# aayush9400/3D-Condtional-Stable-Diffusion

Measured on AMD Instinct MI355X. Metric: latent volumes/sec at 32^3x8ch T=1000 DDPM, higher is better.
Workload: dtype f32 (f16 hi+lo x3 MFMA, f32 accumulate)

## Files before the change

### 3d-condtional-stable-diffusion_amd/_lib.py

```python
from __future__ import annotations

import ctypes as C
import os

_HERE = os.path.dirname(os.path.abspath(__file__))
LIB_PATH = os.environ.get("DM3D_LIB") or os.path.join(_HERE, "csrc", "libdm3d_hip.so")

ACT_NONE, ACT_RELU, ACT_SILU = 0, 1, 2
ABI_VERSION = 111
PREC_F32, PREC_H3 = 0, 1
WL_TAP, WL_PAIR = 0, 1
FMT_F32, FMT_H2 = 0, 1
COUT_PAD, CIN_PAD = 64, 16

_f32p = C.c_void_p
_i32p = C.c_void_p


class ConvDesc(C.Structure):
    _fields_ = [
        ("x1", _f32p), ("x2", _f32p), ("c1", C.c_int32), ("c2", C.c_int32), ("batch", C.c_int32),
        ("in_d", C.c_int32), ("in_h", C.c_int32), ("in_w", C.c_int32), ("upsample", C.c_int32),
        ("ksize", C.c_int32), ("stride", C.c_int32), ("wpk", _f32p), ("bias", _f32p),
        ("pro_scale", _f32p), ("pro_shift", _f32p), ("vec", _f32p), ("vec_idx", _i32p), ("vec_ld", C.c_int32),
# ... 216 lines not shown
GRADNORM_PARTIAL_BLOCKS = 1024
PAIR_PARTIAL_BLOCKS = 64
SSIM_TILE = 32
EDT_MAX_EXTENT = 512
EDT_SURFACE, EDT_FOREGROUND = 0, 1
CCL_MAX_EXTENT = 512
CCL_BLOCK_VOXELS = 1024
CCL_LARGEST, CCL_MIN_SIZE, CCL_FILL_HOLES = 0, 1, 2
SPLINE_MAX_EXTENT = 512
RESAMPLE_F32, RESAMPLE_F64 = 0, 1
NORM_PARTIAL_BLOCKS = 256
AUG_PARTIAL_BLOCKS = 256
STREAM_AUGMENT = 0xA063
MSSSIM_TILE = (32, 16, 32)

SIGNATURES = {
    "dm3d_version": (C.c_int, []),
    "dm3d_last_error": (C.c_char_p, []),
    "dm3d_device_ok": (C.c_int, []),
    "dm3d_packed_weight_elems": (C.c_int64, [C.c_int32, C.c_int32, C.c_int32]),
    "dm3d_pack_weights": (C.c_int, [_f32p, C.c_int32, C.c_int32, C.c_int32, _f32p, _f32p, C.c_void_p]),
    "dm3d_packed_weight_h3_bytes": (C.c_int64, [C.c_int32, C.c_int32, C.c_int32]),
    "dm3d_pack_weights_h3": (C.c_int, [_f32p, C.c_int32, C.c_int32, C.c_int32, C.c_int32, _f32p, C.c_void_p, C.c_void_p]),
    "dm3d_packed_weight_h3p_bytes": (C.c_int64, [C.c_int32, C.c_int32, C.c_int32]),
    "dm3d_pack_weights_h3p": (C.c_int, [_f32p, C.c_int32, C.c_int32, C.c_int32, C.c_int32, _f32p, C.c_void_p, C.c_int32, C.c_void_p]),
    "dm3d_packed_weight_h3w_bytes": (C.c_int64, [C.c_int32, C.c_int32]),
    "dm3d_pack_weights_h3w": (C.c_int, [_f32p, C.c_int32, C.c_int32, C.c_int32, _f32p, C.c_void_p, C.c_void_p]),
    "dm3d_packed_weight_skip_h3p_bytes": (C.c_int64, [C.c_int32, C.c_int32]),
    "dm3d_pack_weights_skip_h3p": (C.c_int, [_f32p, C.c_int32, C.c_int32, C.c_int32, C.c_void_p, C.c_void_p]),
    "dm3d_pack_weights_skip_h3f": (C.c_int, [_f32p, C.c_int32, C.c_int32, C.c_int32, C.c_void_p, C.c_void_p]),
    "dm3d_conv_scratch_bytes": (C.c_int64, [C.POINTER(ConvDesc)]),
    "dm3d_conv_split_counter_words": (C.c_int32, [C.POINTER(ConvDesc)]),
    "dm3d_conv_tile_form": (C.c_int32, [C.POINTER(ConvDesc)]),
    "dm3d_conv_weight_layout": (C.c_int32, [C.c_int32, C.c_int32, C.c_int32, C.c_int32, C.c_int32]),
    "dm3d_attention_workspace_bytes": (C.c_int64, [C.c_int32, C.c_int32, C.c_int32]),
    "dm3d_attention": (C.c_int, [C.POINTER(AttentionDesc), C.c_void_p, C.c_void_p]),
    "dm3d_attention_group": (C.c_int, [C.POINTER(AttentionDesc), C.c_int32, C.c_void_p, C.c_void_p]),
    "dm3d_packed_weight_up_elems": (C.c_int64, [C.c_int32, C.c_int32]),
    "dm3d_pack_weights_up": (C.c_int, [_f32p, C.c_int32, C.c_int32, _f32p, C.c_void_p]),
    "dm3d_packed_weight_up_h3_bytes": (C.c_int64, [C.c_int32, C.c_int32]),
    "dm3d_pack_weights_up_h3": (C.c_int, [_f32p, C.c_int32, C.c_int32, C.c_int32, C.c_void_p, C.c_void_p]),
    "dm3d_pack_weights_convt": (C.c_int, [_f32p, C.c_int32, C.c_int32, _f32p, C.c_void_p]),
    "dm3d_pack_weights_convt_h3": (C.c_int, [_f32p, C.c_int32, C.c_int32, C.c_int32, C.c_void_p, C.c_void_p]),
    "dm3d_conv3d_ndhwc": (C.c_int, [C.POINTER(ConvDesc), C.c_void_p]),
    "dm3d_gemm_tn": (C.c_int, [C.POINTER(GemmDesc), C.c_void_p]),
    "dm3d_gemm_tn_group": (C.c_int, [C.POINTER(GemmDesc), C.c_int32, C.c_void_p]),
    "dm3d_mlp_fused": (C.c_int, [C.POINTER(MlpDesc), C.c_void_p]),
    "dm3d_pack_mlp_weights": (C.c_int, [C.c_void_p, C.c_int32, C.c_int32, C.c_void_p, C.c_void_p]),
    "dm3d_attn_front": (C.c_int, [C.POINTER(AttnFrontDesc), C.c_void_p]),
    "dm3d_pack_front_weights": (C.c_int, [C.c_void_p, C.c_int32, C.c_int32, C.c_void_p, C.c_void_p]),
    "dm3d_split_h2": (C.c_int, [_f32p, C.c_int64, C.c_int32, C.c_int64, C.c_int32, C.c_void_p, C.c_int64, C.c_void_p]),
    "dm3d_layernorm3_h2": (C.c_int, [_f32p, C.c_int64, C.c_int32, C.c_float] + [_f32p] * 9 + [C.c_void_p]),
    "dm3d_softmax_rows_h2": (C.c_int, [_f32p, C.c_int64, C.c_int32, C.c_int64, C.c_void_p]),
    "dm3d_layernorm3": (C.c_int, [_f32p, C.c_int64, C.c_int32, C.c_float] + [_f32p] * 9 + [C.c_void_p]),
    "dm3d_groupnorm_stats": (C.c_int, [_f32p, C.c_int32, C.c_int64, C.c_int32, C.c_void_p, C.c_int32, C.c_int32, C.c_void_p]),
    "dm3d_groupnorm_finalize": (C.c_int, [C.c_void_p, C.c_int32, C.c_int64, C.c_int32, C.c_int32, C.c_float, _f32p, _f32p, _f32p,
                                           _f32p, C.c_void_p]),
    "dm3d_groupnorm_finalize2": (C.c_int, [C.c_void_p, C.c_int32, C.c_void_p, C.c_int32, C.c_int32, C.c_int64, C.c_int32, C.c_float, _f32p, _f32p,
                                          _f32p, _f32p, C.c_void_p]),
    "dm3d_groupnorm_partials": (C.c_int, [_f32p, C.c_int32, C.c_int64, C.c_int32, C.c_void_p, C.c_void_p]),
    "dm3d_groupnorm_partials_bytes": (C.c_int64, [C.c_int32, C.c_int64, C.c_int32]),
    "dm3d_affine_act_batched": (C.c_int, [_f32p, _f32p, C.c_int32, C.c_int64, C.c_int32, _f32p, _f32p, C.c_int32, C.c_void_p]),
    "dm3d_softmax_rows": (C.c_int, [_f32p, C.c_int64, C.c_int32, C.c_int64, C.c_void_p]),
    "dm3d_affine_act": (C.c_int, [_f32p, _f32p, C.c_int64, C.c_int32, _f32p, _f32p, C.c_int32, C.c_void_p]),
    "dm3d_ddpm_update": (C.c_int, [C.POINTER(DdpmDesc), C.c_void_p]),
    "dm3d_ddim_update": (C.c_int, [C.POINTER(DdimDesc), C.c_void_p]),
# ... 117 lines not shown
```

### 3d-condtional-stable-diffusion_amd/csrc/dm3d_conv.hip

```cpp
#include <algorithm>
#include <cstdlib>
#include "dm3d_conv_args.h"
#include <math.h>

namespace {

template <int TD, int TH, int TW, int S, int KS, int WM, int WN>
__global__ __launch_bounds__(256, 2) void conv3d_igemm_f32(const ConvArgs p) {
    constexpr int CK = 16, LDV = CK + 4, NT = 64;
    constexpr int TM = TD * TH * TW;
    constexpr int HD = (TD - 1) * S + KS, HH = (TH - 1) * S + KS, HW = (TW - 1) * S + KS;
    constexpr int HVOX = HD * HH * HW;
    constexpr int TAPS = KS * KS * KS;
    constexpr int MR = TM / WM / 32, NR = NT / WN / 32;
    constexpr int NTHR = WM * WN * 64;
    constexpr int NSLOT = (HVOX * 4 + NTHR - 1) / NTHR;
    static_assert(NTHR == 256, "kernel assumes 4 waves");
    static_assert(TM % (WM * 32) == 0 && NT % (WN * 32) == 0, "tile split");

    extern __shared__ __attribute__((aligned(16))) float smem[];
    float* lds_in = smem;
    float* lds_w = smem + HVOX * LDV;

    const int tid = threadIdx.x;
// ... 148 lines not shown
#pragma unroll
            for (int r = 0; r < 16; ++r) {
                float v = acc[mr][nr][r] + add;
                if (p.relu) v = fmaxf(v, 0.0f);
                if (p.prelu) { const float al = p.prelu[o[r] % sample_elems]; v = v > 0.0f ? v : al * v; }
                if (p.res) v += rv[r];
                if (p.relu_out) v = fmaxf(v, 0.0f);
                if (ok[r]) p.out[o[r]] = v;
            }
        }
    }
}

template <int TD, int TH, int TW, int S, int KS, int WM, int WN>
int launch_conv(ConvArgs& a, hipStream_t st) {
    constexpr int LDV = 20;
    constexpr int HVOX = ((TD - 1) * S + KS) * ((TH - 1) * S + KS) * ((TW - 1) * S + KS);
    constexpr size_t lds = (size_t)(HVOX * LDV + 2 * 64 * LDV) * sizeof(float);
    a.bd = (a.od + TD - 1) / TD;
    a.bh = (a.oh + TH - 1) / TH;
    a.bw = (a.ow + TW - 1) / TW;
    static std::atomic<bool> attr_set[64] = {};
    if (int dev = dm3d_dyn_lds(lds, attr_set, "conv", &conv3d_igemm_f32<TD, TH, TW, S, KS, WM, WN>); dev < 0) return dev;
    dim3 grid((unsigned)(a.batch * a.bd * a.bh * a.bw), (unsigned)(a.coutpad / 64), a.parity ? 8u : 1u);
    hipLaunchKernelGGL((conv3d_igemm_f32<TD, TH, TW, S, KS, WM, WN>), grid, dim3(256), lds, st, a);
    return dm3d_launch_check("conv3d_igemm_f32");
}

}


struct ConvKnobs {
    bool pair_off; int ksplit_mode; long split_wgs, split_target; int split_minchunks, split_maxparts; bool wino_split_off;
    int v3_td; long wide_wgs; bool wino_off; int wino_minchunks, wino_split_minchunks;
};
static ConvKnobs conv_knobs() {
    auto num = [](const char* name, long dflt) { const char* e = getenv(name); return e ? atol(e) : dflt; };
    auto zero = [](const char* name) { const char* e = getenv(name); return e && e[0] == '0'; };
    static const ConvKnobs once = {
        zero("DM3D_CONV_PAIR"),
        (int)num("DM3D_CONV_KSPLIT", -1),
        num("DM3D_CONV_SPLIT_WGS", 256),
        num("DM3D_CONV_SPLIT_TARGET", 512),
        (int)num("DM3D_CONV_SPLIT_MINCHUNKS", 2),
        (int)num("DM3D_CONV_SPLIT_MAXPARTS", 16),
        zero("DM3D_CONV_WINO_SPLIT"),
        0, 0, false, 0, 0};
    ConvKnobs k = once;
    k.v3_td = (int)num("DM3D_CONV_V3_TD", 0);
    k.wide_wgs = num("DM3D_CONV_WIDE_WGS", 512);
    k.wino_off = zero("DM3D_CONV_WINO");
    k.wino_minchunks = (int)num("DM3D_CONV_WINO_MINCHUNKS", 2);
    k.wino_split_minchunks = (int)num("DM3D_CONV_WINO_SPLIT_MINCHUNKS", 16);
    return k;
}

static long split_tiles(const ConvArgs& a, int td) {
    return (long)a.batch * ((a.od + td - 1) / td) * ((a.oh + 7) / 8) * ((a.ow + 7) / 8) * (a.coutpad / 64) * (a.parity ? 8 : 1);
}

static int direct_ksplit(const ConvArgs& a, const ConvKnobs& K) {
    const long wgs = split_tiles(a, 4);
    if (K.ksplit_mode == 0 || wgs > K.split_wgs || a.nchunks < 4) return 1;
    int best = 1;
    for (int d = 2; d <= K.split_maxparts; ++d) {
        if (a.nchunks % d != 0 || a.nchunks / d < K.split_minchunks) continue;
        best = d;
        if (wgs * d >= K.split_target) break;
    }
    return best;
}

static int winograd_ksplit(const ConvArgs& a, const ConvKnobs& K) {
    if (K.wino_split_off || a.nchunks % 2 != 0 || a.nchunks < K.wino_split_minchunks) return 1;
    const long wgs = (long)a.batch * (a.od / 8) * (a.oh / 8) * (a.ow / 8) * (a.coutpad / 64);
    return wgs <= 128 ? 2 : 1;
}

static bool winograd_serves(const ConvArgs& a, int which, int ksplit, const ConvKnobs& K) {
    if (!a.wpk_wino || which != DM3D_CONV_K3S1 || a.parity || a.cout <= 32) return false;
    if (a.s_npairs > 0) {
        if (!a.swpk_f) return false;
        const long long svox = (long long)a.batch * a.ind * a.inh * a.inw;
        if (svox * (a.sc1 > a.sc2 ? a.sc1 : a.sc2) * 4 >= (1ll << 32)) return false;
    }
    if (a.od % 8 != 0 || a.oh % 8 != 0 || a.ow % 8 != 0 || a.padz != 1 || a.pady != 1 || a.padx != 1) return false;
    if (K.wino_off || a.nchunks < K.wino_minchunks) return false;
// ... 39 lines not shown
    a.prelu = d->prelu_alpha; a.relu_out = d->relu_out;
    a.scratch = d->scratch; a.scratch_bytes = d->scratch_bytes;
    a.split_counters = d->split_counters; a.split_counter_words = d->split_counter_words;
    a.range_flag = d->range_flag; a.range_limit = d->range_limit > 0.0f ? d->range_limit : 65504.0f;
    a.wpk_wino = d->wpk_wino;
    a.x_h2 = d->x1_fmt == DM3D_FMT_H2; a.out_h2 = d->out_fmt == DM3D_FMT_H2;
    a.post_scale = d->post_scale; a.post_shift = d->post_shift;
    if (d->skip_wpk) {
        a.sx1 = d->skip_x1; a.sx2 = d->skip_x2; a.sc1 = d->skip_c1; a.sc2 = d->skip_c2; a.swpk = d->skip_wpk;
        a.s_npairs = (int)(dm3d_round_up(d->skip_c1 + d->skip_c2, 32) / 32);
        a.swpk_f = d->skip_wpk_frag;
    }
    a.batch = d->batch;
    a.out_scale = d->precision == DM3D_PREC_H3 ? ldexpf(1.0f, -d->w_exp) : 1.0f;
    if (par_mode) a.w_parity_stride = d->precision == DM3D_PREC_H3
        ? dm3d_packed_weight_h3_bytes(8, cin, d->cout) / 2 : dm3d_packed_weight_elems(8, cin, d->cout);
    a.gn_stats = d->gn_stats;
    r.a = a;
    r.which = par_mode ? DM3D_CONV_UP
                       : (d->ksize == 1 ? DM3D_CONV_K1 : (d->ksize == 4 ? DM3D_CONV_K4S2 : (d->stride == 2 ? DM3D_CONV_K3S2 : DM3D_CONV_K3S1)));

    if (d->precision != DM3D_PREC_H3) { r.family = DM3D_CONV_FAM_F32; return r; }
    if (dm3d_conv_weight_layout(d->ksize, d->stride, d->upsample, d->transpose, d->cout) != DM3D_WL_PAIR) { r.family = DM3D_CONV_FAM_TAP; return r; }
    const bool wino_geometry = r.which == DM3D_CONV_K3S1 && a.cout > 32 && a.od % 8 == 0 && a.oh % 8 == 0 && a.ow % 8 == 0;
    const int ks_direct = direct_ksplit(a, K), ks_wino = wino_geometry ? winograd_ksplit(a, K) : 1;
    auto bytes = [&](int td, int ks) { return split_tiles(a, td) * ks * (int64_t)(td * 8 * 8 * 64) * (int64_t)sizeof(float); };
    if (winograd_serves(a, r.which, a.split_counters ? ks_wino : 1, K)) {
        r.family = DM3D_CONV_FAM_WINO; r.td = 8; r.nct = 4;
        r.ksplit = a.split_counters ? ks_wino : 1;
    } else {
        r.family = DM3D_CONV_FAM_V3;
        r.nct = (r.which == DM3D_CONV_K3S1 && a.cout <= 32) ? (a.cout <= 16 ? 1 : 2) : 4;
        r.td = r.nct != 4 ? 4 : direct_td(a, K);
        r.ksplit = (r.td == 4 && a.split_counters) ? ks_direct : 1;
    }
    r.tiles = split_tiles(a, r.td);
    r.tile_floats = (long)r.td * 8 * 8 * 64;
    if (r.ksplit > 1) { r.need_words = r.tiles; r.need_bytes = bytes(r.td, r.ksplit); }
    if (d->batch <= 0 || d->cout <= 0 || d->in_d <= 0 || d->in_h <= 0 || d->in_w <= 0) return r;
    if (ks_direct > 1) { r.can_words = split_tiles(a, 4); r.can_bytes = bytes(4, ks_direct); }
    if (ks_wino > 1) { r.can_words = std::max(r.can_words, split_tiles(a, 8)); r.can_bytes = std::max(r.can_bytes, bytes(8, ks_wino)); }
    return r;
}

static int conv_validate(const dm3d_conv_desc* d) {
    DM3D_REQUIRE(d != nullptr, "conv: null descriptor");
    DM3D_REQUIRE(d->x1 && d->wpk && d->out, "conv: x1/wpk/out must be non-null");
    DM3D_REQUIRE(d->ksize == 1 || d->ksize == 3 || (d->ksize == 4 && d->stride == 2), "conv: ksize %d not in {1,3} (4 needs stride 2)", d->ksize);
    DM3D_REQUIRE(d->stride == 1 || d->stride == 2, "conv: stride %d not in {1,2}", d->stride);
    DM3D_REQUIRE(!d->transpose || (d->ksize == 4 && d->stride == 2 && !d->upsample), "conv: transpose needs ksize 4, stride 2, no upsample");
    DM3D_REQUIRE(!(d->upsample && d->stride != 1), "conv: upsample requires stride 1");
    DM3D_REQUIRE(!(d->ksize == 1 && (d->stride != 1 || d->upsample)), "conv: ksize 1 supports stride 1 without upsample only");
    DM3D_REQUIRE(d->batch > 0 && d->in_d > 0 && d->in_h > 0 && d->in_w > 0 && d->cout > 0, "conv: non-positive extent");
    DM3D_REQUIRE(d->c1 > 0 && d->c1 % 4 == 0 && d->c2 >= 0 && d->c2 % 4 == 0, "conv: c1=%d c2=%d must be multiples of 4", d->c1, d->c2);
    DM3D_REQUIRE((d->c2 == 0) == (d->x2 == nullptr), "conv: x2 and c2 must be given together");
    DM3D_REQUIRE(d->c2 == 0 || d->c1 % 16 == 0, "conv: with a second input c1=%d must be a multiple of 16", d->c1);
    DM3D_REQUIRE((d->pro_scale == nullptr) == (d->pro_shift == nullptr), "conv: pro_scale and pro_shift go together");
    DM3D_REQUIRE(!d->vec || d->vec_ld >= d->cout, "conv: vec_ld %d < cout %d", d->vec_ld, d->cout);
    const void* ptrs[] = {d->x1, d->x2, d->wpk, d->pro_scale, d->pro_shift, d->out, d->res};
    for (const void* q : ptrs) DM3D_REQUIRE(dm3d_aligned16(q), "conv: pointer %p is not 16-byte aligned", q);
    const int64_t vox = (int64_t)d->batch * d->in_d * d->in_h * d->in_w;
    DM3D_REQUIRE(vox < (1ll << 31) / 4, "conv: %lld voxels overflow the 32-bit voxel index", (long long)vox);
    DM3D_REQUIRE(d->pro_batch_stride == 0 || (d->pro_batch_stride >= d->c1 + d->c2 && d->pro_batch_stride % 4 == 0),
                 "conv: pro_batch_stride must be 0 or a multiple of 4 >= c1+c2");
    DM3D_REQUIRE((d->split_counters == nullptr) == (d->split_counter_words == 0) && d->split_counter_words >= 0, "conv: split_counters and split_counter_words go together");
    if (d->wpk_wino)
// ... 21 lines not shown
        DM3D_REQUIRE((d->skip_c2 == 0) == (d->skip_x2 == nullptr) && (d->skip_c2 == 0 || d->skip_c1 % 16 == 0), "conv: skip_x2 / skip_c2 go together and need skip_c1 %% 16 == 0");
        DM3D_REQUIRE(dm3d_aligned16(d->skip_x1) && dm3d_aligned16(d->skip_x2) && dm3d_aligned16(d->skip_wpk), "conv: skip pointers must be 16-byte aligned");
        DM3D_REQUIRE(dm3d_aligned16(d->skip_wpk_frag), "conv: skip_wpk_frag must be 16-byte aligned");
    }
    DM3D_REQUIRE(dm3d_aligned16(d->scratch) && d->scratch_bytes >= 0, "conv: scratch must be 16-byte aligned");
    DM3D_REQUIRE(d->precision == DM3D_PREC_F32 || d->precision == DM3D_PREC_H3, "conv: unknown precision %d", d->precision);
    DM3D_REQUIRE(d->w_exp >= -100 && d->w_exp <= 100, "conv: w_exp %d out of range", d->w_exp);
    if (d->gn_stats)
        DM3D_REQUIRE(d->out_fmt == DM3D_FMT_F32 && d->cout % 4 == 0 && dm3d_aligned16(d->gn_stats),
                     "conv: gn_stats needs a float32 output, cout %% 4 == 0 and a 16-byte aligned buffer");
    if (d->precision == DM3D_PREC_H3) {
        const int layout = dm3d_conv_weight_layout(d->ksize, d->stride, d->upsample, d->transpose, d->cout);
        DM3D_REQUIRE(d->w_layout == layout, "conv: w_layout %d but this geometry reads layout %d (dm3d_conv_weight_layout)", d->w_layout, layout);
    }
    return DM3D_OK;
}

extern "C" int dm3d_conv3d_ndhwc(const dm3d_conv_desc* d, void* stream) {
    if (int rc = conv_validate(d)) return rc;
    ConvLaunch r = dm3d_conv_resolve(d);
    hipStream_t st = static_cast<hipStream_t>(stream);
    if (r.family == DM3D_CONV_FAM_WINO) return dm3d_conv_launch_h3w(r, st);
    if (r.family == DM3D_CONV_FAM_V3) return dm3d_conv_launch_h3v3(r, st);
    const int rc = r.family == DM3D_CONV_FAM_TAP ? dm3d_conv_launch_h3(r.a, r.which, st) : dm3d_conv_launch_f32(r.a, r.which, st);
    if (rc != DM3D_OK || !r.a.gn_stats) return rc;
    return dm3d_groupnorm_partials(r.a.out, r.a.batch, (int64_t)r.a.fd * r.a.fh * r.a.fw, r.a.cout, r.a.gn_stats, stream);
}

extern "C" int32_t dm3d_conv_tile_form(const dm3d_conv_desc* d) {
    const ConvLaunch r = dm3d_conv_resolve(d);
    return r.family == DM3D_CONV_FAM_WINO ? 10 : (r.family == DM3D_CONV_FAM_V3 ? r.td : 0);
}

extern "C" int64_t dm3d_conv_scratch_bytes(const dm3d_conv_desc* d) { return dm3d_conv_resolve(d).can_bytes; }

extern "C" int32_t dm3d_conv_split_counter_words(const dm3d_conv_desc* d) { return (int32_t)dm3d_conv_resolve(d).can_words; }

extern "C" int32_t dm3d_conv_weight_layout(int32_t ksize, int32_t stride, int32_t upsample, int32_t transpose, int32_t cout) {
    (void)cout;
    if (conv_knobs().pair_off) return DM3D_WL_TAP;
    if (upsample || transpose) return DM3D_WL_PAIR;
    return (ksize == 3 && stride == 1) ? DM3D_WL_PAIR : DM3D_WL_TAP;
}

int dm3d_conv_launch_f32(ConvArgs& a, int which, hipStream_t st) {
    if (which == DM3D_CONV_UP) return launch_conv<4, 8, 8, 1, 2, 4, 1>(a, st);
    if (which == DM3D_CONV_K1) return launch_conv<4, 8, 8, 1, 1, 4, 1>(a, st);
    if (which == DM3D_CONV_K3S2) return launch_conv<2, 4, 8, 2, 3, 2, 2>(a, st);
    if (which == DM3D_CONV_K4S2) return launch_conv<2, 4, 8, 2, 4, 2, 2>(a, st);
    return launch_conv<4, 8, 8, 1, 3, 4, 1>(a, st);
}
```

### 3d-condtional-stable-diffusion_amd/csrc/dm3d_conv_args.h

```cpp
#pragma once
#include "dm3d_common.h"

struct ConvArgs {
    const float* x1; const float* x2; int c1, c2;
    int ind, inh, inw;
    int lgd, lgh, lgw;
    int od, oh, ow;
    int padz, pady, padx;
    int os;
    int ooz, ooy, oox;
    int fd, fh, fw;
    int parity;
    long w_parity_stride;
    const void* wpk; int cinpad, coutpad;
    const float* bias; const float* pscale; const float* pshift; long pro_bstride;
    const float* vec; const int* vec_idx; int vec_ld;
    int relu; const float* res; float* out; int cout;
    const float* prelu; int relu_out;
    int bd, bh, bw;
    int nchunks;
    int batch;
    float out_scale;
    int ksplit;
    int* split_counters;
    int split_counter_words;
    long split_tile_floats;
    void* scratch; long scratch_bytes;
    const float* post_scale; const float* post_shift;
    int out_h2;
    int x_h2;
    const float* sx1; const float* sx2; int sc1, sc2; const void* swpk; int s_npairs;
    const void* swpk_f;
    const void* wpk_wino;
    int* range_flag; float range_limit;
    float* gn_stats;
    int epi_vec4;
};

enum { DM3D_CONV_K3S1 = 0, DM3D_CONV_K3S2 = 1, DM3D_CONV_K1 = 2, DM3D_CONV_UP = 3, DM3D_CONV_K4S2 = 4 };

enum { DM3D_CONV_FAM_F32 = 0,
       DM3D_CONV_FAM_TAP = 1,
       DM3D_CONV_FAM_V3 = 2,
       DM3D_CONV_FAM_WINO = 3 };

struct ConvLaunch {
    ConvArgs a;
    int which;
    int family;
    int td;
    int nct;
    int ksplit;
    long tiles, tile_floats;
    int64_t need_bytes; long need_words;
    int64_t can_bytes; long can_words;
};
ConvLaunch dm3d_conv_resolve(const dm3d_conv_desc* d);

int dm3d_conv_launch_f32(ConvArgs& a, int which, hipStream_t st);
int dm3d_conv_launch_h3(ConvArgs& a, int which, hipStream_t st);
int dm3d_conv_launch_h3v3(const ConvLaunch& r, hipStream_t st);
int dm3d_conv_launch_h3w(const ConvLaunch& r, hipStream_t st);
struct H3v2Launch { ConvArgs k; bool stats_after; };
int dm3d_h3v2_pre_launch(const ConvLaunch& r, H3v2Launch& L);
int dm3d_h3v2_post_launch(const ConvArgs& a, const H3v2Launch& L, hipStream_t st);
```

### 3d-condtional-stable-diffusion_amd/csrc/dm3d_conv_h3v3.hip

```cpp
#include "dm3d_conv_h3v2_parts.h"
#include "dm3d_frag.h"

using namespace h3v2;

#ifdef DM3D_CLOCK_STAMPS
__device__ unsigned long long* g_dbg_stamps_c = nullptr;
extern "C" int dm3d_debug_set_stamps_conv(void* p) { return (int)hipMemcpyToSymbol(HIP_SYMBOL(g_dbg_stamps_c), &p, sizeof(p)); }
#define STAMP(i) do { const unsigned wg_ = blockIdx.x + gridDim.x * blockIdx.y; \
    if (g_dbg_stamps_c && threadIdx.x == 0 && blockIdx.z == 0 && wg_ < 4096) { \
    g_dbg_stamps_c[wg_ * 32 + (i)] = __builtin_amdgcn_s_memtime(); \
    if ((i) == 0) g_dbg_stamps_c[wg_ * 32 + 24] = __builtin_amdgcn_s_memrealtime(); \
    if ((i) == 20) g_dbg_stamps_c[wg_ * 32 + 26] = __builtin_amdgcn_s_memrealtime(); \
    if ((i) == 29) g_dbg_stamps_c[wg_ * 32 + 25] = __builtin_amdgcn_s_memrealtime(); \
    if ((i) == 1) g_dbg_stamps_c[wg_ * 32 + 30] = __builtin_amdgcn_s_memrealtime(); \
    if ((i) == 28) g_dbg_stamps_c[wg_ * 32 + 31] = __builtin_amdgcn_s_memrealtime(); } } while (0)
#else
#define STAMP(i) do { } while (0)
#endif

namespace {

template <int KS, int MODE, int TD, int NCT = 4>
__global__ __launch_bounds__(TD * 64, 2) void conv3d_igemm_h3v3(const ConvArgs p) {
    constexpr int TH = 8, TW = 8, CK = 16, NT = 64, NTHR = TD * 64;
    constexpr int HD = TD - 1 + KS, HH = TH - 1 + KS, HW = TW - 1 + KS, HWP = 12;
    constexpr int HVOX = HD * HH * HW;
    constexpr int TAPS = KS * KS * KS, TAPSP = (TAPS + 3) / 4 * 4;
    constexpr int NP = TAPSP / 2;
    constexpr int NSLOT = (HVOX * 2 + NTHR - 1) / NTHR;
    constexpr int WPAIR = 2 * NT * REC;
    constexpr int RING = 4;
    constexpr int WSLOT = WPAIR * 2 / 1024 / TD;
    constexpr int SPP = (NSLOT + NP - 3) / (NP - 2);
    constexpr int NREQ = (NSLOT + SPP - 1) / SPP;
    constexpr int CV0 = NP - 1 - NREQ < 8 ? NP - 1 - NREQ : 8;
    static_assert(NREQ <= NP - 2 && CV0 >= 1 && CV0 + NREQ <= NP - 1, "request / conversion schedule of the staging slots");
    static_assert(WPAIR * 2 / 1024 % TD == 0, "a weight pair must be a whole number of 1 KB pieces per wave");

    extern __shared__ __attribute__((aligned(16))) _Float16 smem_v3[];
    _Float16* lds_w = smem_v3;
    _Float16* lds_in = smem_v3 + RING * WPAIR;

    STAMP(0);
    const int tid = threadIdx.x;
    const int lane = tid & 63, wave = tid >> 6;
    const int half = lane >> 5, q = (lane >> 4) & 1, row = lane & 15;

    const int ny = gridDim.y;
    int brick, by;
    {
        const unsigned total = gridDim.x * gridDim.y;
        const unsigned d = blockIdx.x + gridDim.x * blockIdx.y;
        unsigned w = d;
        if ((total & 7u) == 0) w = (d & 7u) * (total >> 3) + (d >> 3);
        brick = (int)(w / (unsigned)ny);
        by = (int)(w - (unsigned)brick * (unsigned)ny);
    }
    const int brick_all = brick;
    const int bpv = p.bd * p.bh * p.bw;
    const int b = brick / bpv;
    brick -= b * bpv;
    const int oz0 = (brick / (p.bh * p.bw)) * TD;
    const int oy0 = ((brick / p.bw) % p.bh) * TH;
    const int ox0 = (brick % p.bw) * TW;
    const int ntiles = p.coutpad / NT;
    const int ntile = by % ntiles, khalf = by / ntiles;
    const int c_lo = khalf * (p.nchunks / p.ksplit), c_hi = c_lo + p.nchunks / p.ksplit;
    int padz = p.padz, pady = p.pady, padx = p.padx, ooz = p.ooz, ooy = p.ooy, oox = p.oox;
    const _Float16* wbase = static_cast<const _Float16*>(p.wpk);
    if (p.parity) {
        const int par = blockIdx.z;
        ooz = par >> 2; ooy = (par >> 1) & 1; oox = par & 1;
        padz = 1 - ooz; pady = 1 - ooy; padx = 1 - oox;
        wbase += (size_t)par * p.w_parity_stride;
// ... 11 lines not shown
            if (iz >= 0 && iz < p.ind && iy >= 0 && iy < p.inh && ix >= 0 && ix < p.inw)
                g = ((b * p.ind + iz) * p.inh + iy) * p.inw + ix;
        }
        gvox[j] = g;
        const int v = (hv / HW) * HWP + hv % HW;
        st_off[j] = hv < HVOX ? v * REC + ((piece ^ swz(v)) << 3) : -1;
    }

    int a_rec = (wave * HH + (row & 3)) * HWP + dx_of_row(row);
    const int b_pos = pi_pos(row);
    const int b_hi = (half * NT + b_pos) * REC + ((q ^ swz(b_pos)) << 3);

    f32x4v acc[4][NCT];
#pragma unroll
    for (int pi = 0; pi < 4; ++pi)
#pragma unroll
        for (int ni = 0; ni < NCT; ++ni) acc[pi][ni] = f32x4v{0.f, 0.f, 0.f, 0.f};

    const auto w_rsrc = __builtin_amdgcn_make_buffer_rsrc(const_cast<_Float16*>(wbase), (short)0, (int)((long)ntiles * p.nchunks * (NP * WPAIR * 2)), 0x00020000);
    const int w_voff = wave * 1024 + lane * 16;
    const unsigned w_tile = (unsigned)__builtin_amdgcn_readfirstlane((ntile * p.nchunks) * (NP * WPAIR * 2));
    const int wave_u = __builtin_amdgcn_readfirstlane(wave);
    const int pq_end = c_hi * NP;
    auto fetch_w = [&](int pq, int slot) {
        const unsigned off = w_tile + (unsigned)__builtin_amdgcn_readfirstlane((pq < pq_end ? pq : pq_end - 1) * (WPAIR * 2));
        char* dst = reinterpret_cast<char*>(lds_w) + __builtin_amdgcn_readfirstlane(slot) * (WPAIR * 2) + wave_u * 1024;
#pragma unroll
        for (int i = 0; i < WSLOT; ++i)
            __builtin_amdgcn_raw_ptr_buffer_load_lds(w_rsrc, (__attribute__((address_space(3))) void*)(dst + i * (TD * 1024)), 16, w_voff,
                                                     (int)(off + i * (TD * 1024)), 0, 0);
    };
    int pq = c_lo * NP;
    int ws = 0;
#pragma unroll
    for (int i = 0; i < RING; ++i) fetch_w(pq + i, i);

    constexpr bool pro = MODE == 1, xh2 = MODE == 2;
    f32x4 raw0[NSLOT], raw1[NSLOT];
    f32x4 sc0 = {1.f, 1.f, 1.f, 1.f}, sc1 = sc0, sh0 = {0.f, 0.f, 0.f, 0.f}, sh1 = sh0;
    bool ok0 = false, ok1 = false;
    auto load_halo_slot = [&](int ch, int j) {
        if (xh2) {
            const char* qp = reinterpret_cast<const char*>(p.x1) + (size_t)ch * 64 + piece * 16 + (size_t)(gvox[j] >= 0 ? gvox[j] : 0) * ((size_t)p.c1 * 4);
            raw0[j] = *reinterpret_cast<const f32x4*>(qp);
            raw1[j] = *reinterpret_cast<const f32x4*>(qp + 32);
            return;
        }
        const int c0 = ch * CK;
        const float* src;
        int ldc, cb;
        if (c0 < p.c1) { src = p.x1; ldc = p.c1; cb = c0; } else { src = p.x2; ldc = p.c2; cb = c0 - p.c1; }
        const int cpos = cb + piece * 8;
        const int off0 = cpos < ldc ? cpos : 0, off1 = cpos + 4 < ldc ? cpos + 4 : 0;
        const float* qp = src + (size_t)(gvox[j] >= 0 ? gvox[j] : 0) * ldc;
        raw0[j] = *reinterpret_cast<const f32x4*>(qp + off0);
        raw1[j] = *reinterpret_cast<const f32x4*>(qp + off1);
    };
    constexpr int PLOADS = pro ? 4 : 0;
    auto load_chunk_params = [&](int ch) {
        if (xh2) return;
        const int c0 = ch * CK;
        const int ldc = c0 < p.c1 ? p.c1 : p.c2, cpos = (c0 < p.c1 ? c0 : c0 - p.c1) + piece * 8;
        ok0 = cpos < ldc;
        ok1 = cpos + 4 < ldc;
        if (pro) {
            const int s0 = ok0 ? c0 + piece * 8 : 0, s1 = ok1 ? c0 + piece * 8 + 4 : 0;
            const size_t bo = (size_t)b * p.pro_bstride;
            sc0 = *reinterpret_cast<const f32x4*>(p.pscale + bo + s0);
// ... 64 lines not shown
        o1 = v1 * REC + ((q ^ swz(v1)) << 3);
    };
    const unsigned in_addr = (unsigned)(size_t)(__attribute__((address_space(3))) _Float16*)lds_in;
    const unsigned w_addr = (unsigned)(size_t)(__attribute__((address_space(3))) _Float16*)lds_w;
#define DM3D_DSR(dst, addr, off) asm volatile("ds_read_b128 %0, %1 offset:%2" : "=v"(dst) : "v"(addr), "n"(off))
    auto read_ah = [&](const int pp) {
        int o0, o1; a_offs(pp, o0, o1);
        const unsigned a0 = in_addr + o0 * 2, a1 = in_addr + o1 * 2;
        DM3D_DSR(ah[0], a0, 0); DM3D_DSR(ah[1], a1, 0); DM3D_DSR(ah[2], a0, 48 * REC * 2); DM3D_DSR(ah[3], a1, 48 * REC * 2);
    };
    auto read_al = [&](const int pp) {
        int o0, o1; a_offs(pp, o0, o1);
        const unsigned a0 = in_addr + (o0 ^ 16) * 2, a1 = in_addr + (o1 ^ 16) * 2;
        DM3D_DSR(al[0], a0, 0); DM3D_DSR(al[1], a1, 0); DM3D_DSR(al[2], a0, 48 * REC * 2); DM3D_DSR(al[3], a1, 48 * REC * 2);
    };
    auto read_bh = [&](int slot) {
        const unsigned wa = w_addr + (slot * WPAIR + b_hi) * 2;
        DM3D_DSR(bh[0], wa, 0);
        if constexpr (NCT >= 2) DM3D_DSR(bh[1], wa, 16 * REC * 2);
        if constexpr (NCT == 4) { DM3D_DSR(bh[2], wa, 32 * REC * 2); DM3D_DSR(bh[3], wa, 48 * REC * 2); }
    };
    auto read_bl = [&](int slot) {
        const unsigned wa = w_addr + (slot * WPAIR + (b_hi ^ 16)) * 2;
        DM3D_DSR(bl[0], wa, 0);
        if constexpr (NCT >= 2) DM3D_DSR(bl[1], wa, 16 * REC * 2);
        if constexpr (NCT == 4) { DM3D_DSR(bl[2], wa, 32 * REC * 2); DM3D_DSR(bl[3], wa, 48 * REC * 2); }
    };
#define DM3D_PASS(A, B)                                                                                          \
    _Pragma("unroll") for (int pi_ = 0; pi_ < 4; ++pi_)                                                        \
        _Pragma("unroll") for (int ni_ = 0; ni_ < NCT; ++ni_)                                                  \
            acc[pi_][ni_] = __builtin_amdgcn_mfma_f32_16x16x32_f16(A[pi_], B[ni_], acc[pi_][ni_], 0, 0, 0)

    read_al(0);
    read_bh(0);
    STAMP(1);

    for (int ch = c_lo; ch < c_hi; ++ch) {
        asm volatile("" : "+v"(a_rec));
        const int ch_next = ch + 1 < c_hi ? ch + 1 : ch;
#pragma unroll
        for (int pp = 0; pp < NP; ++pp) {
            const bool last = pp == NP - 1;
            const int ws1 = (ws + 1) & (RING - 1);
            read_ah(pp);
            read_bl(ws);
            __builtin_amdgcn_sched_barrier(0);
            asm volatile("s_waitcnt lgkmcnt(%0)" :: "n"(4 + NCT) : "memory");
            __builtin_amdgcn_sched_barrier(0);
            DM3D_PASS(al, bh);
            __builtin_amdgcn_sched_barrier(0);
            {
                constexpr int DMA_BEHIND = 2 * WSLOT;
                const int extra = halo_ops(pp - 3) + halo_ops(pp - 2) + halo_ops(pp - 1);
#define DM3D_WAIT_VM_LGKM0(n) __builtin_amdgcn_s_waitcnt((((n) & 15) | (7 << 4) | ((((n) >> 4) & 3) << 14)))
                switch (extra) {
                case 0:  DM3D_WAIT_VM_LGKM0(DMA_BEHIND); break;
                case 2:  DM3D_WAIT_VM_LGKM0(DMA_BEHIND + 2); break;
                case 4:  DM3D_WAIT_VM_LGKM0(DMA_BEHIND + 4); break;
                case 6:  DM3D_WAIT_VM_LGKM0(DMA_BEHIND + 6); break;
                case 8:  DM3D_WAIT_VM_LGKM0(DMA_BEHIND + 8); break;
                case 10: DM3D_WAIT_VM_LGKM0(DMA_BEHIND + 10); break;
                case 12: DM3D_WAIT_VM_LGKM0(DMA_BEHIND + 12); break;
                case 14: DM3D_WAIT_VM_LGKM0(DMA_BEHIND + 14); break;
                case 16: DM3D_WAIT_VM_LGKM0(DMA_BEHIND + 16); break;
                default: DM3D_WAIT_VM_LGKM0(0); break;
                }
#undef DM3D_WAIT_VM_LGKM0
                __builtin_amdgcn_s_barrier();
                asm volatile("" ::: "memory");
// ... 37 lines not shown
            DM3D_PASS(ah, bl);
            __builtin_amdgcn_sched_barrier(0);
            if (last) {
                lds_barrier();
                read_al(0);
                __builtin_amdgcn_sched_barrier(0);
            }
            ws = ws1;
            ++pq;
        }
    }
#undef DM3D_PASS
#undef DM3D_DSR
    STAMP(28);
    asm volatile("s_waitcnt vmcnt(0) lgkmcnt(0)" ::: "memory");
    __builtin_amdgcn_s_barrier();
    asm volatile("" ::: "memory");

    const Brick br = {b, oz0, oy0, ox0, ooz, ooy, oox, ntile, khalf};
    if constexpr (KS == 3 && NCT == 4) {
        skip_phase<TD>(p, smem_v3, acc, br);
    }
    STAMP(19);
    if (p.ksplit > 1) {
        const long tile = ((long)blockIdx.z * gridDim.x + brick_all) * ntiles + ntile;
        const SplitTile stile = split_tile(p, tile, khalf);
        split_store(stile, acc, 0);
        STAMP(20);
        if (!split_is_last(p, tile, reinterpret_cast<unsigned*>(smem_v3))) return;
        STAMP(21);
        split_gather(stile, p, khalf, acc, 0);
        STAMP(22);
    }
    if (p.gn_stats) {
        float gn[NCT * 8];
#pragma unroll
        for (int i = 0; i < NCT * 8; ++i) gn[i] = 0.0f;
        epilogue<TD, NCT>(p, acc, br, -1, 4, -1, gn);
        gn_flush<TD, NCT>(p, gn, br, threadIdx.x >> 6, 1);
    } else {
        epilogue<TD, NCT>(p, acc, br);
    }
    STAMP(29);
}

template <int KS, int MODE, int TD, int NCT = 4>
int launch_v3(const ConvLaunch& r, hipStream_t st) {
    constexpr int HREC = (TD - 1 + KS) * (7 + KS) * 12;
    constexpr int main_halfs = HREC * REC + 4 * 2 * 64 * REC, skip_halfs = (KS == 3 && NCT == 4) ? skip_lds_halfs<TD>() : 0;
    constexpr size_t lds = (size_t)(main_halfs > skip_halfs ? main_halfs : skip_halfs) * sizeof(_Float16);
    static_assert((TD == 4 ? 2 : 1) * lds <= 160 * 1024, "workgroups per CU x LDS");
    static std::atomic<bool> attr_set[64] = {};
    if (int dev = dm3d_dyn_lds(lds, attr_set, "conv", &conv3d_igemm_h3v3<KS, MODE, TD, NCT>); dev < 0) return dev;
    H3v2Launch L;
    if (int rc = dm3d_h3v2_pre_launch(r, L)) return rc;
    const ConvArgs& k = L.k;
    dim3 grid((unsigned)(k.batch * k.bd * k.bh * k.bw), (unsigned)(k.coutpad / 64 * k.ksplit), k.parity ? 8u : 1u);
    hipLaunchKernelGGL((conv3d_igemm_h3v3<KS, MODE, TD, NCT>), grid, dim3(TD * 64), lds, st, k);
    if (int rc = dm3d_launch_check("conv3d_igemm_h3v3")) return rc;
    return dm3d_h3v2_post_launch(r.a, L, st);
}

template <int KS, int MODE>
int launch_td(const ConvLaunch& r, hipStream_t st) {
    if constexpr (KS == 3) {
        if (r.nct != 4) {
            DM3D_REQUIRE(r.a.s_npairs == 0 && !r.a.out_h2, "conv: the fused skip conv / hand-off output need cout > 32");
            return r.nct == 1 ? launch_v3<KS, MODE, 4, 1>(r, st) : launch_v3<KS, MODE, 4, 2>(r, st);
        }
    }
    return r.td == 8 ? launch_v3<KS, MODE, 8>(r, st) : launch_v3<KS, MODE, 4>(r, st);
}

}

int dm3d_conv_launch_h3v3(const ConvLaunch& r, hipStream_t st) {
    const ConvArgs& a = r.a;
    if (r.which == DM3D_CONV_UP) return a.pscale ? launch_td<2, 1>(r, st) : launch_td<2, 0>(r, st);
    if (a.x_h2) return launch_td<3, 2>(r, st);
    return a.pscale ? launch_td<3, 1>(r, st) : launch_td<3, 0>(r, st);
}
```

### include/dm3d.h

```cpp
#ifndef DM3D_H
#define DM3D_H

#include <stdint.h>

#ifdef __cplusplus
extern "C" {
#endif

#define DM3D_VERSION 111

#define DM3D_OK            0
#define DM3D_EINVAL       -1
#define DM3D_EUNSUPPORTED -2
#define DM3D_EHIP         -3

#define DM3D_ACT_NONE 0
#define DM3D_ACT_RELU 1
#define DM3D_ACT_SILU 2

#define DM3D_PREC_F32 0
#define DM3D_PREC_H3  1

#define DM3D_FMT_F32 0
#define DM3D_FMT_H2  1
// ... 47 lines not shown
    const float* bias;
    const float* pro_scale;
    const float* pro_shift;
    const float* vec;
    const int32_t* vec_idx;
    int32_t vec_ld;
    int32_t relu;
    const float* res;
    float* out;
    int32_t cout;
    int32_t precision;
    int32_t w_exp;
    const float* prelu_alpha;
    int32_t relu_out;
    int32_t transpose;
    int64_t pro_batch_stride;
    int32_t w_layout;
    const float* skip_x1; const float* skip_x2; int32_t skip_c1, skip_c2; const void* skip_wpk;
    int32_t x1_fmt, out_fmt;
    const float* post_scale; const float* post_shift;
    void* scratch;
    int64_t scratch_bytes;
    int32_t* range_flag; float range_limit;
    const void* wpk_wino;
    const void* skip_wpk_frag;
    float* gn_stats;
    int32_t* split_counters; int32_t split_counter_words;
} dm3d_conv_desc;

int     dm3d_conv3d_ndhwc(const dm3d_conv_desc* d, void* stream);
int64_t dm3d_conv_scratch_bytes(const dm3d_conv_desc* d);
int32_t dm3d_conv_split_counter_words(const dm3d_conv_desc* d);
int32_t dm3d_conv_tile_form(const dm3d_conv_desc* d);

typedef struct dm3d_gemm_desc {
    const float* a; int64_t lda; int64_t stride_a;
    const float* b; int64_t ldb; int64_t stride_b;
    float* out;     int64_t ldo; int64_t stride_o;
    int32_t m, n, k, batch;
    float alpha;
    const float* bias;
    int32_t bias_along_m;
    int32_t act;
    const float* res; int64_t ldr; int64_t stride_r;
    int32_t precision;
    int32_t a_fmt, b_fmt;
    int32_t out_fmt;
    const float* res2;
    int32_t* range_flag; float range_limit;
} dm3d_gemm_desc;

int dm3d_gemm_tn(const dm3d_gemm_desc* d, void* stream);
int dm3d_gemm_tn_group(const dm3d_gemm_desc* descs, int32_t count, void* stream);

int dm3d_pack_mlp_weights(const void* w_h2, int32_t units, int32_t which, void* tiled, void* stream);
typedef struct dm3d_mlp_desc {
    const void* x; int64_t ldx;
    const void* w0; const float* b0;
    const void* w1; const float* b1;
    const float* res; const float* res2; int64_t ldr;
    void* out; int64_t ldo; int32_t out_fmt;
    int32_t m, units;
    int32_t* range_flag; float range_limit;
    const void* w2; const float* b2;
    const float* res3; int64_t ldr3;
} dm3d_mlp_desc;
// ... 470 lines not shown
```

Baseline: 2.466.

## Add operand-swapped narrow-cout conv path with register-held weights and row epilogue

For k3 convolutions with cout of 32 or less, adds a swapped MFMA form where the weights act as the A operand and sit in registers, fetched through a small ring of buffer loads instead of being staged in LDS. This removes the weight LDS region and its barriers and shrinks LDS use. A new row-oriented epilogue writes four output channels per lane with vector stores. It applies only when shapes and pointers are aligned, and adds register pressure plus a new code path that can be switched off with an environment knob.

```diff
diff --git a/3d-condtional-stable-diffusion_amd/_lib.py b/3d-condtional-stable-diffusion_amd/_lib.py
--- a/3d-condtional-stable-diffusion_amd/_lib.py
+++ b/3d-condtional-stable-diffusion_amd/_lib.py
@@ -272,6 +272,7 @@
     "dm3d_conv_scratch_bytes": (C.c_int64, [C.POINTER(ConvDesc)]),
     "dm3d_conv_split_counter_words": (C.c_int32, [C.POINTER(ConvDesc)]),
     "dm3d_conv_tile_form": (C.c_int32, [C.POINTER(ConvDesc)]),
+    "dm3d_conv_operand_swapped": (C.c_int32, [C.POINTER(ConvDesc)]),
     "dm3d_conv_weight_layout": (C.c_int32, [C.c_int32, C.c_int32, C.c_int32, C.c_int32, C.c_int32]),
     "dm3d_attention_workspace_bytes": (C.c_int64, [C.c_int32, C.c_int32, C.c_int32]),
     "dm3d_attention": (C.c_int, [C.POINTER(AttentionDesc), C.c_void_p, C.c_void_p]),
diff --git a/3d-condtional-stable-diffusion_amd/csrc/dm3d_conv.hip b/3d-condtional-stable-diffusion_amd/csrc/dm3d_conv.hip
--- a/3d-condtional-stable-diffusion_amd/csrc/dm3d_conv.hip
+++ b/3d-condtional-stable-diffusion_amd/csrc/dm3d_conv.hip
@@ -204,7 +204,7 @@
 
 struct ConvKnobs {
     bool pair_off; int ksplit_mode; long split_wgs, split_target; int split_minchunks, split_maxparts; bool wino_split_off;
-    int v3_td; long wide_wgs; bool wino_off; int wino_minchunks, wino_split_minchunks;
+    int v3_td; long wide_wgs; bool wino_off; int wino_minchunks, wino_split_minchunks; bool swap_off;
 };
 static ConvKnobs conv_knobs() {
     auto num = [](const char* name, long dflt) { const char* e = getenv(name); return e ? atol(e) : dflt; };
@@ -217,14 +217,21 @@
         (int)num("DM3D_CONV_SPLIT_MINCHUNKS", 2),
         (int)num("DM3D_CONV_SPLIT_MAXPARTS", 16),
         zero("DM3D_CONV_WINO_SPLIT"),
-        0, 0, false, 0, 0};
+        0, 0, false, 0, 0, false};
     ConvKnobs k = once;
     k.v3_td = (int)num("DM3D_CONV_V3_TD", 0);
     k.wide_wgs = num("DM3D_CONV_WIDE_WGS", 512);
     k.wino_off = zero("DM3D_CONV_WINO");
     k.wino_minchunks = (int)num("DM3D_CONV_WINO_MINCHUNKS", 2);
     k.wino_split_minchunks = (int)num("DM3D_CONV_WINO_SPLIT_MINCHUNKS", 16);
+    k.swap_off = zero("DM3D_CONV_NARROW_SWAP");
     return k;
+}
+
+static bool swapped_serves(const ConvArgs& a, const ConvKnobs& K) {
+    auto al16 = [](const void* q) { return (reinterpret_cast<size_t>(q) & 15) == 0; };
+    if (K.swap_off || a.od % 4 != 0 || a.oh % 8 != 0 || a.ow % 8 != 0 || a.cout % 4 != 0 || a.prelu) return false;
+    return al16(a.out) && al16(a.res) && al16(a.bias) && al16(a.vec) && (a.vec == nullptr || a.vec_ld % 4 == 0);
 }
 
 static long split_tiles(const ConvArgs& a, int td) {
@@ -330,6 +337,7 @@
         r.family = DM3D_CONV_FAM_V3;
         r.nct = (r.which == DM3D_CONV_K3S1 && a.cout <= 32) ? (a.cout <= 16 ? 1 : 2) : 4;
         r.td = r.nct != 4 ? 4 : direct_td(a, K);
+        r.swapped = r.nct != 4 && swapped_serves(a, K);
         r.ksplit = (r.td == 4 && a.split_counters) ? ks_direct : 1;
     }
     r.tiles = split_tiles(a, r.td);
@@ -417,6 +425,8 @@
     return r.family == DM3D_CONV_FAM_WINO ? 10 : (r.family == DM3D_CONV_FAM_V3 ? r.td : 0);
 }
 
+extern "C" int32_t dm3d_conv_operand_swapped(const dm3d_conv_desc* d) { return dm3d_conv_resolve(d).swapped; }
+
 extern "C" int64_t dm3d_conv_scratch_bytes(const dm3d_conv_desc* d) { return dm3d_conv_resolve(d).can_bytes; }
 
 extern "C" int32_t dm3d_conv_split_counter_words(const dm3d_conv_desc* d) { return (int32_t)dm3d_conv_resolve(d).can_words; }
diff --git a/3d-condtional-stable-diffusion_amd/csrc/dm3d_conv_args.h b/3d-condtional-stable-diffusion_amd/csrc/dm3d_conv_args.h
--- a/3d-condtional-stable-diffusion_amd/csrc/dm3d_conv_args.h
+++ b/3d-condtional-stable-diffusion_amd/csrc/dm3d_conv_args.h
@@ -50,6 +50,7 @@
     int family;
     int td;
     int nct;
+    int swapped;
     int ksplit;
     long tiles, tile_floats;
     int64_t need_bytes; long need_words;
diff --git a/3d-condtional-stable-diffusion_amd/csrc/dm3d_conv_h3v3.hip b/3d-condtional-stable-diffusion_amd/csrc/dm3d_conv_h3v3.hip
--- a/3d-condtional-stable-diffusion_amd/csrc/dm3d_conv_h3v3.hip
+++ b/3d-condtional-stable-diffusion_amd/csrc/dm3d_conv_h3v3.hip
@@ -20,7 +20,57 @@
 
 namespace {
 
-template <int KS, int MODE, int TD, int NCT = 4>
+template <int TD, int NRT>
+__device__ __forceinline__ void epilogue_rows(const ConvArgs& p, f32x4v (&acc)[4][NRT], const Brick& br) {
+    const int lane = threadIdx.x & 63, wave = threadIdx.x >> 6;
+    const int row = lane & 15, g4 = lane >> 4;
+    const int vrow = p.vec ? (p.vec_idx ? p.vec_idx[br.b] : br.b) : 0;
+    const size_t zbase = (((size_t)br.b * p.fd + br.oz0 + wave) * p.fh) * p.fw * p.cout;
+    float* outz = p.out + zbase;
+    const float* resz = p.res ? p.res + zbase : nullptr;
+    const int vox0 = (br.oy0 + (row & 3)) * p.fw + br.ox0 + dx_of_row(row);
+    const f32x4 zero = {0.f, 0.f, 0.f, 0.f};
+    bool live[NRT];
+    int o0[NRT];
+    f32x4 add_t[NRT], rv4[NRT][4];
+#pragma unroll
+    for (int t = 0; t < NRT; ++t) {
+        const int n = t * 16 + g4 * 4;
+        live[t] = n < p.cout;
+        const int nc = live[t] ? n : 0;
+        o0[t] = vox0 * p.cout + nc;
+        add_t[t] = p.bias ? *reinterpret_cast<const f32x4*>(p.bias + nc) : zero;
+        if (p.vec) {
+            const f32x4 vv = *reinterpret_cast<const f32x4*>(p.vec + (size_t)vrow * p.vec_ld + nc);
+#pragma unroll
+            for (int j = 0; j < 4; ++j) add_t[t][j] += vv[j];
+        }
+        if (resz) {
+#pragma unroll
+            for (int pi = 0; pi < 4; ++pi) rv4[t][pi] = *reinterpret_cast<const f32x4*>(resz + o0[t] + (4 * (pi >> 1) * p.fw + 4 * (pi & 1)) * p.cout);
+        }
+    }
+    float amax = 0.0f;
+#pragma unroll
+    for (int t = 0; t < NRT; ++t)
+#pragma unroll
+        for (int pi = 0; pi < 4; ++pi) {
+            f32x4 v4;
+#pragma unroll
+            for (int j = 0; j < 4; ++j) {
+                float v = fmaf(acc[pi][t][j], p.out_scale, add_t[t][j]);
+                if (p.relu) v = fmaxf(v, 0.0f);
+                if (resz) v += rv4[t][pi][j];
+                if (p.relu_out) v = fmaxf(v, 0.0f);
+                if (live[t]) DM3D_AMAX(amax, v);
+                v4[j] = v;
+            }
+            if (live[t]) *reinterpret_cast<f32x4*>(outz + o0[t] + (4 * (pi >> 1) * p.fw + 4 * (pi & 1)) * p.cout) = v4;
+        }
+    if (p.range_flag && amax > p.range_limit) *p.range_flag = 1;
+}
+
+template <int KS, int MODE, int TD, int NCT = 4, bool SWAP = false>
 __global__ __launch_bounds__(TD * 64, 2) void conv3d_igemm_h3v3(const ConvArgs p) {
     constexpr int TH = 8, TW = 8, CK = 16, NT = 64, NTHR = TD * 64;
     constexpr int HD = TD - 1 + KS, HH = TH - 1 + KS, HW = TW - 1 + KS, HWP = 12;
@@ -39,7 +89,7 @@
 
     extern __shared__ __attribute__((aligned(16))) _Float16 smem_v3[];
     _Float16* lds_w = smem_v3;
-    _Float16* lds_in = smem_v3 + RING * WPAIR;
+    _Float16* lds_in = smem_v3 + (SWAP ? 0 : RING * WPAIR);
 
     STAMP(0);
     const int tid = threadIdx.x;
@@ -117,8 +167,24 @@
     };
     int pq = c_lo * NP;
     int ws = 0;
-#pragma unroll
-    for (int i = 0; i < RING; ++i) fetch_w(pq + i, i);
+    constexpr int WD = SWAP ? (NCT == 1 ? 7 : 2) : 1;
+    static_assert(!SWAP || (KS == 3 && NCT <= 2 && NP % WD == 0), "the swapped form: k3, one or two row tiles, a ring that divides the pairs of a chunk");
+    h8 wh[WD][NCT], wl[WD][NCT];
+    auto fetch_wr = [&](int pq_, const int slot) {
+        const int off = (int)w_tile + __builtin_amdgcn_readfirstlane((pq_ < pq_end ? pq_ : pq_end - 1) * (WPAIR * 2));
+#pragma unroll
+        for (int t = 0; t < NCT; ++t) {
+            wh[slot][t] = __builtin_bit_cast(h8, __builtin_amdgcn_raw_buffer_load_b128(w_rsrc, (b_hi + t * 16 * REC) * 2, off, 0));
+            wl[slot][t] = __builtin_bit_cast(h8, __builtin_amdgcn_raw_buffer_load_b128(w_rsrc, ((b_hi ^ 16) + t * 16 * REC) * 2, off, 0));
+        }
+    };
+    if constexpr (SWAP) {
+#pragma unroll
+        for (int i = 0; i < WD; ++i) fetch_wr(pq + i, i);
+    } else {
+#pragma unroll
+        for (int i = 0; i < RING; ++i) fetch_w(pq + i, i);
+    }
 
     constexpr bool pro = MODE == 1, xh2 = MODE == 2;
     f32x4 raw0[NSLOT], raw1[NSLOT];
@@ -249,9 +315,69 @@
             acc[pi_][ni_] = __builtin_amdgcn_mfma_f32_16x16x32_f16(A[pi_], B[ni_], acc[pi_][ni_], 0, 0, 0)
 
     read_al(0);
-    read_bh(0);
+    if constexpr (!SWAP) read_bh(0);
     STAMP(1);
 
+    if constexpr (SWAP) {
+#define DM3D_PASS_SW(W, X)                                                                                       \
+    _Pragma("unroll") for (int pi_ = 0; pi_ < 4; ++pi_)                                                        \
+        _Pragma("unroll") for (int t_ = 0; t_ < NCT; ++t_)                                                     \
+            acc[pi_][t_] = __builtin_amdgcn_mfma_f32_16x16x32_f16(W[t_], X[pi_], acc[pi_][t_], 0, 0, 0)
+        h8 xh[2][4];
+        auto read_xh = [&](const int pp_, const int buf) {
+            int o0, o1; a_offs(pp_, o0, o1);
+            const unsigned a0 = in_addr + o0 * 2, a1 = in_addr + o1 * 2;
+            DM3D_DSR(xh[buf][0], a0, 0); DM3D_DSR(xh[buf][1], a1, 0); DM3D_DSR(xh[buf][2], a0, 48 * REC * 2); DM3D_DSR(xh[buf][3], a1, 48 * REC * 2);
+        };
+        read_xh(0, 0);
+        for (int ch = c_lo; ch < c_hi; ++ch) {
+            asm volatile("" : "+v"(a_rec));
+            const int ch_next = ch + 1 < c_hi ? ch + 1 : ch;
+#pragma unroll
+            for (int pp = 0; pp < NP; ++pp) {
+                const bool last = pp == NP - 1;
+                const int s = pp % WD, xb = pp & 1;
+                if (!last) read_xh(pp + 1, xb ^ 1);
+                __builtin_amdgcn_sched_barrier(0);
+                if (!last) {
+                    asm volatile("s_waitcnt lgkmcnt(4)" ::: "memory");
+                } else {
+                    __builtin_amdgcn_s_waitcnt(0xC07F);
+                    __builtin_amdgcn_s_barrier();
+                    asm volatile("" ::: "memory");
+                }
+                __builtin_amdgcn_sched_barrier(0);
+                DM3D_PASS_SW(wh[s], al);
+                __builtin_amdgcn_sched_barrier(0);
+                if (pp < NREQ) {
+#pragma unroll
+                    for (int j = pp * SPP; j < (pp + 1) * SPP && j < NSLOT; ++j) load_halo_slot(ch_next, j);
+                }
+                if (pp == 0) load_chunk_params(ch_next);
+                if (!last) read_al(pp + 1);
+                else store_image();
+                __builtin_amdgcn_sched_barrier(0);
+                DM3D_PASS_SW(wh[s], xh[xb]);
+                __builtin_amdgcn_sched_barrier(0);
+                if (pp >= CV0 && pp < CV0 + NREQ) {
+#pragma unroll
+                    for (int j = (pp - CV0) * SPP; j < (pp - CV0 + 1) * SPP && j < NSLOT; ++j) convert_slot(j);
+                }
+                __builtin_amdgcn_sched_barrier(0);
+                DM3D_PASS_SW(wl[s], xh[xb]);
+                __builtin_amdgcn_sched_barrier(0);
+                fetch_wr(pq + WD, s);
+                if (last) {
+                    lds_barrier();
+                    read_al(0);
+                    read_xh(0, 0);
+                    __builtin_amdgcn_sched_barrier(0);
+                }
+                ++pq;
+            }
+        }
+#undef DM3D_PASS_SW
+    } else
     for (int ch = c_lo; ch < c_hi; ++ch) {
         asm volatile("" : "+v"(a_rec));
         const int ch_next = ch + 1 < c_hi ? ch + 1 : ch;
@@ -355,6 +481,9 @@
         split_gather(stile, p, khalf, acc, 0);
         STAMP(22);
     }
+    if constexpr (SWAP) {
+        epilogue_rows<TD, NCT>(p, acc, br);
+    } else
     if (p.gn_stats) {
         float gn[NCT * 8];
 #pragma unroll
@@ -367,19 +496,19 @@
     STAMP(29);
 }
 
-template <int KS, int MODE, int TD, int NCT = 4>
+template <int KS, int MODE, int TD, int NCT = 4, bool SWAP = false>
 int launch_v3(const ConvLaunch& r, hipStream_t st) {
     constexpr int HREC = (TD - 1 + KS) * (7 + KS) * 12;
-    constexpr int main_halfs = HREC * REC + 4 * 2 * 64 * REC, skip_halfs = (KS == 3 && NCT == 4) ? skip_lds_halfs<TD>() : 0;
+    constexpr int main_halfs = HREC * REC + (SWAP ? 0 : 4 * 2 * 64 * REC), skip_halfs = (KS == 3 && NCT == 4) ? skip_lds_halfs<TD>() : 0;
     constexpr size_t lds = (size_t)(main_halfs > skip_halfs ? main_halfs : skip_halfs) * sizeof(_Float16);
     static_assert((TD == 4 ? 2 : 1) * lds <= 160 * 1024, "workgroups per CU x LDS");
     static std::atomic<bool> attr_set[64] = {};
-    if (int dev = dm3d_dyn_lds(lds, attr_set, "conv", &conv3d_igemm_h3v3<KS, MODE, TD, NCT>); dev < 0) return dev;
+    if (int dev = dm3d_dyn_lds(lds, attr_set, "conv", &conv3d_igemm_h3v3<KS, MODE, TD, NCT, SWAP>); dev < 0) return dev;
     H3v2Launch L;
     if (int rc = dm3d_h3v2_pre_launch(r, L)) return rc;
     const ConvArgs& k = L.k;
     dim3 grid((unsigned)(k.batch * k.bd * k.bh * k.bw), (unsigned)(k.coutpad / 64 * k.ksplit), k.parity ? 8u : 1u);
-    hipLaunchKernelGGL((conv3d_igemm_h3v3<KS, MODE, TD, NCT>), grid, dim3(TD * 64), lds, st, k);
+    hipLaunchKernelGGL((conv3d_igemm_h3v3<KS, MODE, TD, NCT, SWAP>), grid, dim3(TD * 64), lds, st, k);
     if (int rc = dm3d_launch_check("conv3d_igemm_h3v3")) return rc;
     return dm3d_h3v2_post_launch(r.a, L, st);
 }
@@ -389,6 +518,7 @@
     if constexpr (KS == 3) {
         if (r.nct != 4) {
             DM3D_REQUIRE(r.a.s_npairs == 0 && !r.a.out_h2, "conv: the fused skip conv / hand-off output need cout > 32");
+            if (r.swapped) return r.nct == 1 ? launch_v3<KS, MODE, 4, 1, true>(r, st) : launch_v3<KS, MODE, 4, 2, true>(r, st);
             return r.nct == 1 ? launch_v3<KS, MODE, 4, 1>(r, st) : launch_v3<KS, MODE, 4, 2>(r, st);
         }
     }
diff --git a/include/dm3d.h b/include/dm3d.h
--- a/include/dm3d.h
+++ b/include/dm3d.h
@@ -103,6 +103,7 @@
 int64_t dm3d_conv_scratch_bytes(const dm3d_conv_desc* d);
 int32_t dm3d_conv_split_counter_words(const dm3d_conv_desc* d);
 int32_t dm3d_conv_tile_form(const dm3d_conv_desc* d);
+int32_t dm3d_conv_operand_swapped(const dm3d_conv_desc* d);
 
 typedef struct dm3d_gemm_desc {
     const float* a; int64_t lda; int64_t stride_a;
```

Result: no change. 2.474 (median of 6 runs) (+0.3%).
